# Chrissie-Law/Causal-Domain-Clustering-for-Multi-Domain-Recommendation

Measured on AMD Instinct MI355X. Metric: train samples/sec + AUC parity, PLE 3-domain batch 4096 at 1/2/4/8 MI355X, higher is better.
Workload: dtype bf16; 1 GPU; PLE 3-domain full training step (fwd + BCE + whole-table L2 + bwd + Adam), 26 fields x vocab 1000000, emb_dim=16, batch 4096/GPU; global_batch=4096, table_mode=lazy, hip_graph=True, row_sort_one_batch_ahead=True, id_dist=uniform, parallelism=dp1, attention_branch=False, full=False, steady_state=True, preroll_steps=1785, flush_every=64

## Files before the change

causal-domain-clustering-for-multi-domain-recommendation_amd/_lib.py:

```python
import ctypes as C
import os

from . import build as _build

MAX_GROUPS = 32
MAX_TENSORS = 48
MAX_GATES = 16
MAX_SEL = 16
MAX_BN_SEGS = 24
SORT_MAX_B = 16384
SORT_MAX_ROWS = 32768
BN_ROWS_PER_BLOCK = 64
ROWDOT_PARTS = 256
PREC_BF16 = 0
PREC_F32 = 1

c_f = C.c_float
c_i32 = C.c_int32
c_i64 = C.c_int64
c_p = C.c_void_p


class AdamHP(C.Structure):
    _fields_ = [("lerp_w", c_f), ("beta2", c_f), ("one_minus_beta2", c_f), ("eps", c_f),
# ... 317 lines not shown
    "cdc_embed_index": (c_i32, [c_p, c_p, c_p, c_p, c_i64, c_i32, c_i64, c_p]),
    "cdc_embed_sort_dedupe": (c_i32, [c_p, c_p, c_p, c_p, c_p, c_p, c_i64, c_i32, c_p]),
    "cdc_embed_sort_dedupe_ids": (c_i32, [c_p, c_p, c_i64, c_p, c_p, c_i32, c_p, c_p, c_p, c_p, c_p, c_p, c_i64, c_i32, c_p]),
    "cdc_embed_segment_sum": (c_i32, [c_p, c_p, c_p, c_p, c_p, c_p, c_i64, c_i32, c_i32, c_p]),
    "cdc_embed_segment_sum_direct": (c_i32, [c_p, c_p, c_p, c_p, c_p, c_p, c_i64, c_i32, c_i32, c_p]),
    "cdc_embed_segsum_lazy_update": (c_i32, [c_p, c_p, c_p, c_p, c_p, c_p, c_p, c_p, c_p, AdamHP, c_p, c_i64, c_i32, c_i32, c_i32, c_p]),
    "cdc_embed_grad_dense": (c_i32, [c_p, c_p, c_p, c_p, c_i64, c_i32, c_i32, c_i64, c_p]),
    "cdc_embed_adam_touched": (c_i32, [c_p, c_p, c_p, c_p, c_p, c_p, c_p, AdamHP, c_p, c_i64, c_i32, c_i32, c_p]),
    "cdc_embed_adam_dense_pass": (c_i32, [c_p, c_p, c_p, c_i64, AdamHP, c_p, c_p, c_p]),
    "cdc_embed_adam_patch": (c_i32, [c_p, c_p, c_p, c_p, c_p, c_p, c_i64, c_i32, c_i32, c_p]),
    "cdc_embed_lazy_catchup": (c_i32, [c_p, c_p, c_p, c_p, c_p, c_p, AdamHP, c_p, c_p, c_i32, c_i64, c_i32, c_i32, c_p]),
    "cdc_embed_lazy_catchup_gather": (c_i32, [c_p, c_p, c_p, c_p, c_p, c_p, c_p, c_p, AdamHP, c_p, c_p, c_p, c_i64, c_i64, c_i32, c_i32, c_p]),
    "cdc_embed_lazy_update": (c_i32, [c_p, c_p, c_p, c_p, c_p, c_p, c_p, AdamHP, c_p, c_p, c_i32, c_i64, c_i32, c_i32, c_p]),
    "cdc_embed_lazy_flush": (c_i32, [c_p, c_p, c_p, c_p, c_i64, c_i32, AdamHP, c_p, c_i32, c_i32, c_i32, c_i32, c_p]),
    "cdc_embed_lazy_flush_bg": (c_i32, [c_p, c_p, c_p, c_p, c_i64, c_i32, AdamHP, c_p, c_i32, c_i32, c_i32, c_i32, c_i32, c_p]),
    "cdc_embed_merge_dedupe": (c_i32, [c_p, c_p, c_p, c_p, c_p, c_p, c_i64, c_i32, c_i32, c_p]),
    "cdc_eval_workspace_bytes": (c_i64, [c_i64, c_i32]),
    "cdc_eval_metrics": (c_i32, [c_p, c_p, c_p, c_i64, c_i64, c_i32, c_p, c_p, c_p, c_p, c_i64, c_p]),
    "cdc_shard_bucket": (c_i32, [c_p, c_p, c_p, c_p, c_p, c_i64, c_i32, c_i32, c_i32, c_p]),
    "cdc_shard_expand": (c_i32, [c_p, c_p, c_p, c_p, c_p, c_p, c_p, c_i64, c_i32, c_i32, c_i32, c_i32, c_p]),
    "cdc_shard_pack": (c_i32, [c_p, c_p, c_p, c_p, c_p, c_i64, c_i32, c_i32, c_i32, c_i32, c_p]),
    "cdc_glinear_fwd": (c_i32, [C.POINTER(LinFwdArgs), c_i32, c_p]),
    "cdc_glinear_bwd_x": (c_i32, [C.POINTER(LinBwdxArgs), c_i32, c_p]),
    "cdc_transpose_multi": (c_i32, [C.POINTER(TransposeArgs), c_p]),
    "cdc_gemm_bf16_nt": (c_i32, [C.POINTER(G2Args), c_p]),
    "cdc_weight_shadows": (c_i32, [C.POINTER(WShadowArgs), c_p]),
    "cdc_shadow_bf16": (c_i32, [C.POINTER(ShadowArgs), c_p]),
    "cdc_glinear_bwd_w": (c_i32, [C.POINTER(LinBwdwArgs), c_i32, c_p]),
    "cdc_glinear_bwd_w_pair": (c_i32, [C.POINTER(LinBwdwArgs), C.POINTER(LinBwdwArgs), c_p, c_p]),
    "cdc_glinear_bwd_w_pair_reduce": (c_i32, [C.POINTER(LinBwdwArgs), C.POINTER(LinBwdwArgs), c_p, c_p]),
# ... 137 lines not shown
```

causal-domain-clustering-for-multi-domain-recommendation_amd/csrc/common.h:

```cpp
#pragma once
#include <hip/hip_runtime.h>
#include <stdint.h>
#include <stdio.h>
#include "cdcmdr.h"

#define CDC_WAVE 64

void cdc_set_error(const char* fmt, ...);

#define CDC_CHECK_ARG(cond, code, ...)            \
    do {                                          \
        if (!(cond)) {                            \
            cdc_set_error(__VA_ARGS__);           \
            return (code);                        \
        }                                         \
    } while (0)

#define CDC_LAUNCH_CHECK(name)                                                     \
    do {                                                                           \
        hipError_t e__ = hipGetLastError();                                        \
        if (e__ != hipSuccess) {                                                   \
            cdc_set_error("%s: launch failed: %s", name, hipGetErrorString(e__)); \
            return (int)e__;                                                       \
        }                                                                          \
// ... 111 lines not shown
        }
    }
}
__device__ __forceinline__ void adam_scaled_step_pk(cdc_f2& w, cdc_f2& M, cdc_f2& V, float beta1, float beta2, float C1, float C2) {
    M = __builtin_elementwise_fma((cdc_f2){beta1, beta1}, M, w);
    V = __builtin_elementwise_fma((cdc_f2){beta2, beta2}, V, w * w);
    cdc_f2 sq;
    sq.x = __builtin_amdgcn_sqrtf(V.x);
    sq.y = __builtin_amdgcn_sqrtf(V.y);
    const cdc_f2 d = __builtin_elementwise_fma(sq, (cdc_f2){C1, C1}, (cdc_f2){C2, C2});
    cdc_f2 r;
    r.x = __builtin_amdgcn_rcpf(d.x);
    r.y = __builtin_amdgcn_rcpf(d.y);
    w = __builtin_elementwise_fma(M, r, w);
}
template <int N>
__device__ __forceinline__ void adam_replay_wave_scaled(float (&w)[N], float (&m)[N], float (&v)[N], int from, int to, const cdc_adam_hp& hp) {
    static_assert(N % 2 == 0, "pairs of elements");
    const int last_i = hp.n_scalars - 1;
    const float A_conv = hp.replay_tab[2 * last_i], E_conv = hp.replay_tab[2 * last_i + 1];
    const float beta1 = 1.f - hp.lerp_w;
    int fmin = from < to ? from : to;
#pragma unroll
    for (int o = 32; o > 0; o >>= 1) {
        const int other = __shfl_xor(fmin, o, 64);
        fmin = other < fmin ? other : fmin;
    }
    fmin = __builtin_amdgcn_readfirstlane(fmin);
    if (fmin >= to) return;
    const float ik1 = hp.ik1, ik2 = hp.ik2;
    cdc_f2 W[N / 2], M[N / 2], V[N / 2];
#pragma unroll
    for (int k = 0; k < N / 2; ++k) {
        W[k] = (cdc_f2){w[2 * k], w[2 * k + 1]};
        M[k] = (cdc_f2){m[2 * k], m[2 * k + 1]} * ik1;
        V[k] = (cdc_f2){v[2 * k], v[2 * k + 1]} * ik2;
    }
    for (int s = fmin + 1; s <= to; ++s) {
        float A = A_conv, E = E_conv;
        if (s < last_i) { A = hp.replay_tab[2 * s]; E = hp.replay_tab[2 * s + 1]; }
        if (s > from) {
#pragma unroll
            for (int k = 0; k < N / 2; ++k) adam_scaled_step_pk(W[k], M[k], V[k], beta1, hp.beta2, A, E);
        }
    }
    if (from < to) {
#pragma unroll
        for (int k = 0; k < N / 2; ++k) {
            const cdc_f2 mo = __builtin_elementwise_fma(M[k], (cdc_f2){hp.k1, hp.k1}, M[k] * hp.k1_lo);
            const cdc_f2 vo = __builtin_elementwise_fma(V[k], (cdc_f2){hp.k2, hp.k2}, V[k] * hp.k2_lo);
            w[2 * k] = W[k].x; w[2 * k + 1] = W[k].y;
            m[2 * k] = mo.x; m[2 * k + 1] = mo.y;
            v[2 * k] = vo.x; v[2 * k + 1] = vo.y;
        }
    }
}

template <bool FAST, int N>
__device__ __forceinline__ void adam_replay_wave(float (&w)[N], float (&m)[N], float (&v)[N], int from, int to, const AdamConsts& c,
                                                 const cdc_adam_hp& hp) {
    if constexpr (FAST && N % 2 == 0) {
        if (hp.replay_tab && hp.k1 > 0.f && hp.k2 > 0.f) {
            adam_replay_wave_scaled<N>(w, m, v, from, to, hp);
            return;
        }
    }
    const int last_i = hp.n_scalars - 1;
    const float ss_conv = hp.step_scalars[2 * last_i];
    const float bc_conv = FAST ? hp.inv_bc2[last_i] : hp.step_scalars[2 * last_i + 1];
    int fmin = from < to ? from : to;
#pragma unroll
    for (int o = 32; o > 0; o >>= 1) {
        const int other = __shfl_xor(fmin, o, 64);
        fmin = other < fmin ? other : fmin;
    }
    fmin = __builtin_amdgcn_readfirstlane(fmin);
    for (int s = fmin + 1; s <= to; ++s) {
        float ss = ss_conv, bc = bc_conv;
        if (s < last_i) {
            ss = hp.step_scalars[2 * s];
            bc = FAST ? hp.inv_bc2[s] : hp.step_scalars[2 * s + 1];
        }
        if (s > from) {
            if constexpr (FAST && N % 2 == 0) {
#pragma unroll
                for (int k = 0; k < N; k += 2) {
                    cdc_f2 w2 = {w[k], w[k + 1]}, m2 = {m[k], m[k + 1]}, v2 = {v[k], v[k + 1]};
                    adam_elem_fast_pk(w2, m2, v2, c, ss, bc);
                    w[k] = w2.x; w[k + 1] = w2.y; m[k] = m2.x; m[k + 1] = m2.y; v[k] = v2.x; v[k + 1] = v2.y;
                }
            } else {
#pragma unroll
                for (int k = 0; k < N; ++k) {
                    if (FAST) adam_elem_fast(w[k], m[k], v[k], c, ss, bc);
                    else adam_elem(w[k], m[k], v[k], 0.f, c, ss, bc);
                }
            }
// ... 55 lines not shown
```

causal-domain-clustering-for-multi-domain-recommendation_amd/csrc/embedding.hip:

```cpp
#include "common.h"
#include "adam_dense.h"

template <int VEC>
__global__ void __launch_bounds__(256) k_gather_fwd(const int32_t* __restrict__ ids, const int32_t* __restrict__ offsets,
                                                    const float* __restrict__ table, float* __restrict__ out,
                                                    __bf16* __restrict__ out_h, int64_t ld_out_h,
                                                    int32_t* __restrict__ idx_out, int32_t* __restrict__ err_flag,
                                                    int64_t n_pos, int32_t F, int32_t D, int64_t R) {
    CDC_PRIO_MAIN();
    const int chunks = D / VEC;
    const int64_t total = n_pos * chunks;
    for (int64_t i = (int64_t)blockIdx.x * blockDim.x + threadIdx.x; i < total; i += (int64_t)gridDim.x * blockDim.x) {
        const int64_t pos = i / chunks;
        const int c = (int)(i - pos * chunks);
        const int f = (int)(pos % F);
        const int32_t row = (int32_t)((uint32_t)ids[pos] + (uint32_t)offsets[f]);
        const bool ok = row >= 0 && (int64_t)row < R;
        if (c == 0 && idx_out) idx_out[pos] = ok ? row : -1;
        if (!ok && c == 0 && err_flag) atomicMax(err_flag, (int32_t)(pos < 0x7ffffffe ? pos + 1 : 0x7fffffff));
        if (VEC == 4) {
            float4 val = make_float4(0.f, 0.f, 0.f, 0.f);
            if (ok) val = *reinterpret_cast<const float4*>(table + (int64_t)row * D + c * 4);
            *reinterpret_cast<float4*>(out + pos * D + c * 4) = val;
            if (out_h) {
// ... 1242 lines not shown
                  CDC_E_BADARG, "embed_lazy_update: null pointer");
    CDC_CHECK_ARG(B > 0 && F > 0 && D > 0, CDC_E_BADARG, "embed_lazy_update: bad sizes");
    const bool vec = (D % 4 == 0) && ((((uintptr_t)w | (uintptr_t)m | (uintptr_t)v | (uintptr_t)rowgrad) & 15) == 0);
    const int64_t total = (int64_t)F * B * (vec ? D / 4 : D);
    int blocks = (int)std::min<int64_t>(cdc_ceil_div(total, 256), 256 * 16);
    if (vec)
        hipLaunchKernelGGL(k_lazy_update<4>, dim3(blocks), dim3(256), 0, (hipStream_t)stream, rowgrad, uniq_row, uniq_cnt, w, m, v, last, hp,
                           step_dev, (int32_t)B, F, D);
    else
        hipLaunchKernelGGL(k_lazy_update<1>, dim3(blocks), dim3(256), 0, (hipStream_t)stream, rowgrad, uniq_row, uniq_cnt, w, m, v, last, hp,
                           step_dev, (int32_t)B, F, D);
    CDC_LAUNCH_CHECK("embed_lazy_update");
    return 0;
}

template <bool FAST, int VEC>
__global__ void __launch_bounds__(256) __attribute__((amdgpu_waves_per_eu(8, 8))) k_lazy_flush(float* __restrict__ w, float* __restrict__ m, float* __restrict__ v,
                                                    int32_t* __restrict__ last, int64_t R, int32_t D, cdc_adam_hp hp,
                                                    const int32_t* __restrict__ step_dev, int32_t step_bias, int32_t period,
                                                    int32_t own_mod, int32_t own_rem, int32_t mark, int64_t win_lo, int64_t win_n) {
    const int target = *step_dev + step_bias;
    int64_t row_lo = 0, row_hi = R;
    if (period > 1) {
        const int64_t rps = (R + period - 1) / period;
        row_lo = (int64_t)(((target % period) + period) % period) * rps;
        row_hi = row_lo + rps < R ? row_lo + rps : R;
        if (row_lo >= row_hi) return;
    }
    if (win_lo > row_lo) row_lo = win_lo;
    if (win_lo + win_n < row_hi) row_hi = win_lo + win_n;
    if (row_lo >= row_hi) return;
    const AdamConsts c = make_consts(hp);
    const int64_t stride = own_mod > 1 ? own_mod : 1;
    int64_t first = row_lo;
    if (stride > 1) first = row_lo + ((own_rem - row_lo % stride) + stride) % stride;
    if (first >= row_hi) return;
    const int64_t n_rows = (row_hi - first + stride - 1) / stride;
    const int chunks = D / VEC;
    const int64_t total = n_rows * chunks;
    typedef float f4v __attribute__((ext_vector_type(4)));
    const int32_t itotal = (int32_t)total;
    auto row_of = [&](int32_t i) -> int64_t { return first + (int64_t)(i / chunks) * stride; };
    auto fetch = [&](int32_t i, int& from, float (&wv)[VEC], float (&mv)[VEC], float (&vv)[VEC]) __attribute__((always_inline)) {
        const bool in = i < itotal;
        const int64_t row = in ? row_of(i) : first;
        from = in ? last[row] : target;
        const bool act = in && from < target;
        if (!act) from = target;
#pragma unroll
        for (int k = 0; k < VEC; ++k) { wv[k] = 0.f; mv[k] = 0.f; vv[k] = 1.f; }
        if (act) {
            const int64_t e0 = row * D + (i % chunks) * VEC;
            if (VEC == 4) {
                const f4v a4 = __builtin_nontemporal_load(reinterpret_cast<const f4v*>(w + e0)),
                          b4 = __builtin_nontemporal_load(reinterpret_cast<const f4v*>(m + e0)),
                          c4 = __builtin_nontemporal_load(reinterpret_cast<const f4v*>(v + e0));
#pragma unroll
                for (int k = 0; k < 4; ++k) { wv[k] = a4[k]; mv[k] = b4[k]; vv[k] = c4[k]; }
            } else {
                wv[0] = w[e0]; mv[0] = m[e0]; vv[0] = v[e0];
            }
        }
    };
    const int32_t gstride = (int32_t)(gridDim.x * blockDim.x);
    int cfrom, nfrom;
    float cw[VEC], cm[VEC], cv[VEC], nw[VEC], nm[VEC], nv[VEC];
    int32_t i = (int32_t)(blockIdx.x * blockDim.x + threadIdx.x);
    fetch(i, cfrom, cw, cm, cv);
    for (int32_t base = (int32_t)(blockIdx.x * blockDim.x); base < itotal; base += gstride, i += gstride) {
        fetch(base + gstride < itotal ? i + gstride : itotal, nfrom, nw, nm, nv);
        const bool act = cfrom < target;
        if (__any(act)) {
            adam_replay_wave<FAST, VEC>(cw, cm, cv, cfrom, target, c, hp);
            if (act) {
                const int64_t row = row_of(i);
                const int64_t e0 = row * D + (i % chunks) * VEC;
                if (VEC == 4) {
                    __builtin_nontemporal_store((f4v){cw[0], cw[1], cw[2], cw[3]}, reinterpret_cast<f4v*>(w + e0));
                    __builtin_nontemporal_store((f4v){cm[0], cm[1], cm[2], cm[3]}, reinterpret_cast<f4v*>(m + e0));
                    __builtin_nontemporal_store((f4v){cv[0], cv[1], cv[2], cv[3]}, reinterpret_cast<f4v*>(v + e0));
                } else {
                    w[e0] = cw[0]; m[e0] = cm[0]; v[e0] = cv[0];
                }
                if (mark && (i % chunks) == 0) last[row] = target;
            }
        }
        cfrom = nfrom;
#pragma unroll
        for (int k = 0; k < VEC; ++k) { cw[k] = nw[k]; cm[k] = nm[k]; cv[k] = nv[k]; }
    }
}
__global__ void __launch_bounds__(256) k_lazy_set_last(int32_t* __restrict__ last, int64_t R, const int32_t* __restrict__ step_dev,
                                                       int32_t step_bias, int32_t period, int32_t own_mod, int32_t own_rem) {
    const int target = *step_dev + step_bias;
    int64_t row_lo = 0, row_hi = R;
    if (period > 1) {
        const int64_t rps = (R + period - 1) / period;
        row_lo = (int64_t)(((target % period) + period) % period) * rps;
        row_hi = row_lo + rps < R ? row_lo + rps : R;
    }
    for (int64_t i = row_lo + (int64_t)blockIdx.x * blockDim.x + threadIdx.x; i < row_hi; i += (int64_t)gridDim.x * blockDim.x) {
        if (own_mod > 1 && (i % own_mod) != own_rem) continue;
        if (last[i] < target) last[i] = target;
    }
}

static int lazy_flush_launch(float* w, float* m, float* v, int32_t* last, int64_t R, int32_t D, cdc_adam_hp hp,
                             const int32_t* step_dev, int32_t step_bias, int32_t period, int32_t own_mod, int32_t own_rem,
                             int32_t waves_per_simd, void* stream) {
    CDC_CHECK_ARG(w && m && v && last && step_dev && hp.step_scalars && hp.n_scalars > 0, CDC_E_BADARG, "embed_lazy_flush: null pointer");
    CDC_CHECK_ARG(R > 0 && D > 0 && period >= 0 && own_mod >= 0 && (own_mod <= 1 || (own_rem >= 0 && own_rem < own_mod)), CDC_E_BADARG,
                  "embed_lazy_flush: bad sizes");
    CDC_CHECK_ARG(!hp.fast_replay || hp.inv_bc2, CDC_E_BADARG, "embed_lazy_flush: fast_replay needs the inv_bc2 table");
    const bool vec = (D % 4 == 0) && ((((uintptr_t)w | (uintptr_t)m | (uintptr_t)v) & 15) == 0);
    int64_t rows_call = period > 1 ? cdc_ceil_div(R, period) : R;
    if (own_mod > 1) rows_call = cdc_ceil_div(rows_call, own_mod) + 1;
    int blocks = (int)std::max<int64_t>(1, std::min<int64_t>(cdc_ceil_div(rows_call * D / (vec ? 4 : 1), 256), 256 * 16));
    if (waves_per_simd > 0) {
        static int n_cu = 0;
        if (n_cu == 0) {
            int dev = 0, v_ = 0;
            if (hipGetDevice(&dev) != hipSuccess || hipDeviceGetAttribute(&v_, hipDeviceAttributeMultiprocessorCount, dev) != hipSuccess || v_ <= 0) v_ = 256;
            n_cu = v_;
        }
        const int64_t cap = (int64_t)waves_per_simd * n_cu;
        if (blocks > cap) blocks = (int)cap;
    }
    hipStream_t st = (hipStream_t)stream;
    const int32_t chunks = vec ? D / 4 : D;
    const int32_t mark = (64 % chunks == 0) ? 1 : 0;
    const int64_t max_items = ((int64_t)1 << 31) - 1 - (int64_t)blocks * 256 - 256;
    const int64_t win_rows = std::max<int64_t>(1, max_items / chunks);
    CDC_CHECK_ARG(period <= 1 || rows_call <= win_rows, CDC_E_TOOBIG,
                  "embed_lazy_flush: a slice of %lld rows x %d chunks exceeds the 2^31 work items of one launch (raise flush_every)",
                  (long long)rows_call, (int)chunks);
    for (int64_t lo = 0; lo < R; lo += (period > 1 ? R : win_rows)) {
        const int64_t n = period > 1 ? R : std::min<int64_t>(win_rows, R - lo);
        if (hp.fast_replay) {
            if (vec) hipLaunchKernelGGL((k_lazy_flush<true, 4>), dim3(blocks), dim3(256), 0, st, w, m, v, last, R, D, hp, step_dev, step_bias, period, own_mod, own_rem, mark, lo, n);
            else     hipLaunchKernelGGL((k_lazy_flush<true, 1>), dim3(blocks), dim3(256), 0, st, w, m, v, last, R, D, hp, step_dev, step_bias, period, own_mod, own_rem, mark, lo, n);
        } else {
            if (vec) hipLaunchKernelGGL((k_lazy_flush<false, 4>), dim3(blocks), dim3(256), 0, st, w, m, v, last, R, D, hp, step_dev, step_bias, period, own_mod, own_rem, mark, lo, n);
            else     hipLaunchKernelGGL((k_lazy_flush<false, 1>), dim3(blocks), dim3(256), 0, st, w, m, v, last, R, D, hp, step_dev, step_bias, period, own_mod, own_rem, mark, lo, n);
        }
    }
    CDC_LAUNCH_CHECK("embed_lazy_flush");
    if (!mark) {
        int blocks2 = (int)std::max<int64_t>(1, std::min<int64_t>(cdc_ceil_div(period > 1 ? cdc_ceil_div(R, period) : R, 256), 256 * 16));
        hipLaunchKernelGGL(k_lazy_set_last, dim3(blocks2), dim3(256), 0, (hipStream_t)stream, last, R, step_dev, step_bias, period, own_mod, own_rem);
        CDC_LAUNCH_CHECK("embed_lazy_set_last");
    }
    return 0;
}
extern "C" int cdc_embed_lazy_flush(float* w, float* m, float* v, int32_t* last, int64_t R, int32_t D, cdc_adam_hp hp,
                                    const int32_t* step_dev, int32_t step_bias, int32_t period, int32_t own_mod, int32_t own_rem,
                                    void* stream) {
    return lazy_flush_launch(w, m, v, last, R, D, hp, step_dev, step_bias, period, own_mod, own_rem, 0, stream);
}
extern "C" int cdc_embed_lazy_flush_bg(float* w, float* m, float* v, int32_t* last, int64_t R, int32_t D, cdc_adam_hp hp,
                                       const int32_t* step_dev, int32_t step_bias, int32_t period, int32_t own_mod, int32_t own_rem,
                                       int32_t waves_per_simd, void* stream) {
    return lazy_flush_launch(w, m, v, last, R, D, hp, step_dev, step_bias, period, own_mod, own_rem, waves_per_simd, stream);
}


#define SHARD_MAX_RANKS 16
__global__ void __launch_bounds__(SORT_THREADS) k_shard_bucket(const int32_t* __restrict__ uniq_row, const int32_t* __restrict__ uniq_cnt,
                                                               int32_t* __restrict__ send_ids, int32_t* __restrict__ slot_of,
                                                               int32_t* __restrict__ overflow, int32_t B, int32_t F, int32_t n_rank,
                                                               int32_t cap) {
    __shared__ int32_t wave_tot[SORT_THREADS / 64];
    const int f = blockIdx.x, o = blockIdx.y, tid = threadIdx.x;
    const int n = uniq_cnt[f];
    const int per = (B + SORT_THREADS - 1) / SORT_THREADS;
    const int begin = tid * per;
    const int32_t* ur = uniq_row + (int64_t)f * B;
    int local = 0;
// ... 119 lines not shown
```

causal-domain-clustering-for-multi-domain-recommendation_amd/optim.py:

```python
import ctypes as C
import math

import os

import torch

from . import _lib as L


def step_scalar_table(lr, beta1, beta2, n=4096, truncate=False):
    rows = [(0.0, 1.0)]
    for t in range(1, n):
        rows.append((lr / (1.0 - beta1 ** t), math.sqrt(1.0 - beta2 ** t)))
    tab = torch.tensor(rows, dtype=torch.float64).to(torch.float32)
    if truncate:
        same = (tab == tab[-1]).all(dim=1)
        first = int(torch.nonzero(~same).max().item()) + 1 if bool((~same).any()) else 0
        tab = tab[:first + 1].contiguous()
    return tab


class FusedAdam:
    def __init__(self, model, lr=1e-3, betas=(0.9, 0.99), eps=1e-8, weight_decay=1e-8, table_mode="dense", frozen=(),
                 fast_replay=True, flush_every=64):
# ... 117 lines not shown
    def flush_slice(self, background_waves=0):
        if self.table_mode != "lazy" or self.flush_every <= 1:
            return
        nb = 24.0 * self.table.numel() / self.flush_every / max(self.own_mod, 1)
        if background_waves > 0:
            L.launch("cdc_embed_lazy_flush(slice)", self.lib.cdc_embed_lazy_flush_bg,
                     (self.table.data_ptr(), self.table_m.data_ptr(), self.table_v.data_ptr(), self.table_last.data_ptr(),
                      self.table.shape[0], self.table.shape[1], self._hp(), self.step_dev.data_ptr(), -1, self.flush_every,
                      self.own_mod, self.own_rem, int(background_waves)), self._stream(), nbytes=nb)
            return
        L.launch("cdc_embed_lazy_flush(slice)", self.lib.cdc_embed_lazy_flush,
                 (self.table.data_ptr(), self.table_m.data_ptr(), self.table_v.data_ptr(), self.table_last.data_ptr(),
                  self.table.shape[0], self.table.shape[1], self._hp(), self.step_dev.data_ptr(), -1, self.flush_every,
                  self.own_mod, self.own_rem), self._stream(), nbytes=nb)

    def catchup(self, B, F, D, tag=""):
        assert self.table_mode == "lazy"
        ws = self._workspace(B, F, D, tag)
        L.launch("cdc_embed_lazy_catchup", self.lib.cdc_embed_lazy_catchup,
                 (ws["uniq"].data_ptr(), ws["cnt"].data_ptr(), self.table.data_ptr(), self.table_m.data_ptr(),
                  self.table_v.data_ptr(), self.table_last.data_ptr(), self._hp(), self.step_dev.data_ptr(), None, 0, B, F, D), self._stream())

    def catchup_gather(self, B, F, D, tag, out_ptr, out_h, ld_out_h):
        assert self.table_mode == "lazy"
        ws = self._workspace(B, F, D, tag)
        L.launch("cdc_embed_lazy_catchup_gather", self.lib.cdc_embed_lazy_catchup_gather,
                 (ws["uniq"].data_ptr(), ws["cnt"].data_ptr(), ws["seg"].data_ptr(), ws["perm"].data_ptr(), self.table.data_ptr(),
                  self.table_m.data_ptr(), self.table_v.data_ptr(), self.table_last.data_ptr(), self._hp(), self.step_dev.data_ptr(),
                  out_ptr, out_h, ld_out_h, B, F, D), self._stream(), nbytes=float(B) * F * (D * 4 + 4 + D * 4))

# ... 191 lines not shown
```

causal-domain-clustering-for-multi-domain-recommendation_amd/trainer.py:

```python
import ctypes as C
import os

import torch

from . import _lib as L
from .optim import FusedAdam


def _run_steps(steps):
    def fn():
        st = C.c_void_p(torch.cuda.current_stream().cuda_stream)
        for s_ in steps:
            s_(st)
    return fn


def _merge_pieces(seq):
    merged = []
    for is_comm, fn in seq:
        if merged and not is_comm and not merged[-1][0]:
            merged[-1][1].append(fn)
        else:
            merged.append((is_comm, [fn]))
    return merged


class TrainStep:

    def __init__(self, model, optimizer: FusedAdam, batch_size, mode="multi", use_graph=False, dist=None, sync_bn=True,
                 table_dist=None, shard_slack=1.5, train_mode=True, overlap=True, overlap_waves=2, sort_ahead=True, fuse_gather=False,
                 defer_dw_reduce=None, global_rows=None, cap_rows=None, tower_one_launch=True, rows_dense_one_launch=True):
        self.model, self.opt, self.B, self.mode = model, optimizer, int(batch_size), mode
        self.lib = L.load()
        self.dist = dist
        self.sync_bn = bool(sync_bn)
        self.world = 1 if dist is None else dist.world_size
        self.dp_on = self.world > 1 or bool(getattr(dist, "force", False))
        self.global_B = self.B * self.world if global_rows is None else int(global_rows)
        self._shard_slack = float(shard_slack)
        dev = optimizer.device
        self.device = dev
        self.train_mode = bool(train_mode)
        self._overlap_ok, self._overlap_waves = bool(overlap), int(overlap_waves)
        self._rows_dense_one = bool(rows_dense_one_launch) and not self.dp_on
        self.tower_one_launch = bool(tower_one_launch)
        self._defer_dw = (not self.dp_on) if defer_dw_reduce is None else (bool(defer_dw_reduce) and not self.dp_on)
        assert mode in ("multi", "single", "mean", "star", "single_group")
        self.holder = self._build_plan()
        self.plan = self.holder.plan
        self.emb = self.holder.emb_op
        self.out = self.holder.outputs[0]
        self.y = torch.zeros(self.B, dtype=torch.int16, device=dev)
        self.group = torch.zeros(self.B, dtype=torch.int64, device=dev) if mode == "multi" else None
        if mode == "single_group":
            self.group_in = self.holder.inputs[1]
        if mode == "star":
            self.group = self.holder.inputs[1]
            self.order = self.holder.extra_outputs[0]
            self.y_perm = torch.zeros(self.B, dtype=torch.int16, device=dev)
# ... 175 lines not shown
            bg, fused = self._overlap_ok, self._fuse_gather_ok
            side = self._side_stream() if bg else main
            if bg:
                side.wait_stream(main)
            with torch.cuda.stream(side):
                if not have:
                    opt.begin_step_sort(emb.ids, emb.offsets, B, F, D, tag=cur, err=emb.err if fused else None, begin=False)
                if fused:
                    oh, ldh = plan.shadow_view(emb.out) if (plan.use_g2 and plan.has_shadow(emb.out)) else (None, 0)
                    opt.catchup_gather(B, F, D, cur, emb.out.ptr, oh, ldh)
                else:
                    opt.catchup(B, F, D, cur)
                if bg:
                    rows_ready = torch.cuda.Event()
                    rows_ready.record(side)
                opt.flush_slice(background_waves=self._overlap_waves if bg else 0)
                if prefetch:
                    opt.begin_step_sort(self.ids_next, emb.offsets, B, F, D, tag=nxt, begin=False)
            nws = plan.n_wshadow_steps
            for fn in plan.fwd_steps[:nws]:
                fn(st)
            if bg:
                main.wait_event(rows_ready)
            for fn in plan.fwd_steps[nws:]:
                if not (fused and fn is emb.fwd_step):
                    fn(st)
            self._bce()
            plan.backward()
            if self._rows_dense_one:
                if bg:
                    main.wait_stream(side)
                opt.rows_and_dense_step(emb.idx, emb.out.grad.root, B, F, D, plan.param_grads, plan._param_refs, plan.grad_slabs, tag=cur)
            else:
# ... 390 lines not shown
```

include/cdcmdr.h:

```cpp
#ifndef CDCMDR_H
#define CDCMDR_H

#include <stdint.h>

#ifdef __cplusplus
extern "C" {
#endif

#define CDC_ABI_VERSION 1

#define CDC_E_BADARG   (-1)
#define CDC_E_TOOBIG   (-2)
#define CDC_E_ALIGN    (-3)

#define CDC_PREC_BF16 0
#define CDC_PREC_F32  1

#define CDC_MAX_GROUPS 32
#define CDC_MAX_TENSORS 48

int cdc_abi_version(void);
const char* cdc_last_error(void);


// ... 52 lines not shown
                          float* w, float* m, float* v, int32_t* last,
                          cdc_adam_hp hp, const int32_t* step_dev, double* reg_ring, int32_t ring_len,
                          int64_t B, int32_t F, int32_t D, void* stream);
int cdc_embed_lazy_catchup_gather(const int32_t* uniq_row, const int32_t* uniq_cnt, const int32_t* seg_start, const int32_t* perm,
                                  float* w, float* m, float* v, int32_t* last, cdc_adam_hp hp, const int32_t* step_dev,
                                  float* out, void* out_h, int64_t ld_out_h, int64_t B, int32_t F, int32_t D, void* stream);
int cdc_embed_segsum_lazy_update(const float* d_out, const int32_t* seg_start, const int32_t* perm, const int32_t* uniq_cnt,
                                 const int32_t* uniq_row, float* w, float* m, float* v, int32_t* last, cdc_adam_hp hp,
                                 const int32_t* step_dev, int64_t B, int32_t F, int32_t D, int32_t short_only, void* stream);
int cdc_embed_lazy_flush(float* w, float* m, float* v, int32_t* last, int64_t R, int32_t D,
                         cdc_adam_hp hp, const int32_t* step_dev, int32_t step_bias, int32_t period,
                         int32_t own_mod, int32_t own_rem, void* stream);
int cdc_embed_lazy_flush_bg(float* w, float* m, float* v, int32_t* last, int64_t R, int32_t D,
                            cdc_adam_hp hp, const int32_t* step_dev, int32_t step_bias, int32_t period,
                            int32_t own_mod, int32_t own_rem, int32_t waves_per_simd, void* stream);

int cdc_embed_merge_dedupe(const int32_t* idx, int32_t* uniq_row, int32_t* seg_start, int32_t* perm, int32_t* uniq_cnt,
                           uint64_t* scratch, int64_t B, int32_t F, int32_t n_runs, void* stream);
int cdc_shard_bucket(const int32_t* uniq_row, const int32_t* uniq_cnt, int32_t* send_ids, int32_t* slot_of, int32_t* overflow,
                     int64_t B, int32_t F, int32_t n_rank, int32_t cap, void* stream);
int cdc_shard_expand(const float* rows_recv, const int32_t* uniq_row, const int32_t* uniq_cnt, const int32_t* seg_start,
                     const int32_t* perm, const int32_t* slot_of, float* out, int64_t B, int32_t F, int32_t D,
                     int32_t n_rank, int32_t cap, void* stream);
int cdc_shard_pack(const float* rowgrad, const int32_t* uniq_row, const int32_t* uniq_cnt, const int32_t* slot_of, float* send,
                   int64_t B, int32_t F, int32_t D, int32_t n_rank, int32_t cap, void* stream);

typedef struct {
    const float* x;  int64_t ldx;
    const float* w;  int64_t ldw;
    const float* bias;
// ... 652 lines not shown
```

Before: 13.10 million samples/s.

## Fuse next-batch sort/dedupe into the background lazy-flush kernel

Adds a combined kernel in which the first F blocks run a register/LDS bitonic sort-dedupe of the next batch's ids at raised priority, while the remaining blocks perform the background lazy Adam flush slice. The flush work is split proportionally between the sort blocks and the others. This replaces the separate flush and sort launches on the side stream. The intent is to save a launch and let the sort overlap the flush inside one grid. It also pins replay scalars to SGPRs and uses shift/mask indexing when chunks is a power of two. The cost is more code paths, a new bitonic sort implementation that must match the old one, and sort blocks that might unbalance the flush.

```diff
diff --git a/causal-domain-clustering-for-multi-domain-recommendation_amd/_lib.py b/causal-domain-clustering-for-multi-domain-recommendation_amd/_lib.py
--- a/causal-domain-clustering-for-multi-domain-recommendation_amd/_lib.py
+++ b/causal-domain-clustering-for-multi-domain-recommendation_amd/_lib.py
@@ -355,6 +355,8 @@
     "cdc_embed_lazy_update": (c_i32, [c_p, c_p, c_p, c_p, c_p, c_p, c_p, AdamHP, c_p, c_p, c_i32, c_i64, c_i32, c_i32, c_p]),
     "cdc_embed_lazy_flush": (c_i32, [c_p, c_p, c_p, c_p, c_i64, c_i32, AdamHP, c_p, c_i32, c_i32, c_i32, c_i32, c_p]),
     "cdc_embed_lazy_flush_bg": (c_i32, [c_p, c_p, c_p, c_p, c_i64, c_i32, AdamHP, c_p, c_i32, c_i32, c_i32, c_i32, c_i32, c_p]),
+    "cdc_embed_lazy_flush_bg_sort": (c_i32, [c_p, c_p, c_p, c_p, c_i64, c_i32, AdamHP, c_p, c_i32, c_i32, c_i32, c_i32, c_i32,
+                                             c_p, c_p, c_p, c_p, c_p, c_p, c_p, c_p, c_i64, c_i32, c_p]),
     "cdc_embed_merge_dedupe": (c_i32, [c_p, c_p, c_p, c_p, c_p, c_p, c_i64, c_i32, c_i32, c_p]),
     "cdc_eval_workspace_bytes": (c_i64, [c_i64, c_i32]),
     "cdc_eval_metrics": (c_i32, [c_p, c_p, c_p, c_i64, c_i64, c_i32, c_p, c_p, c_p, c_p, c_i64, c_p]),
diff --git a/causal-domain-clustering-for-multi-domain-recommendation_amd/csrc/common.h b/causal-domain-clustering-for-multi-domain-recommendation_amd/csrc/common.h
--- a/causal-domain-clustering-for-multi-domain-recommendation_amd/csrc/common.h
+++ b/causal-domain-clustering-for-multi-domain-recommendation_amd/csrc/common.h
@@ -149,7 +149,10 @@
     r.y = __builtin_amdgcn_rcpf(d.y);
     w = __builtin_elementwise_fma(M, r, w);
 }
-template <int N>
+__device__ __forceinline__ float uniform_sgpr(float x) {
+    return __builtin_bit_cast(float, __builtin_amdgcn_readfirstlane(__builtin_bit_cast(int, x)));
+}
+template <int N, bool PIN = false>
 __device__ __forceinline__ void adam_replay_wave_scaled(float (&w)[N], float (&m)[N], float (&v)[N], int from, int to, const cdc_adam_hp& hp) {
     static_assert(N % 2 == 0, "pairs of elements");
     const int last_i = hp.n_scalars - 1;
@@ -174,6 +177,7 @@
     for (int s = fmin + 1; s <= to; ++s) {
         float A = A_conv, E = E_conv;
         if (s < last_i) { A = hp.replay_tab[2 * s]; E = hp.replay_tab[2 * s + 1]; }
+        if constexpr (PIN) { A = uniform_sgpr(A); E = uniform_sgpr(E); }
         if (s > from) {
 #pragma unroll
             for (int k = 0; k < N / 2; ++k) adam_scaled_step_pk(W[k], M[k], V[k], beta1, hp.beta2, A, E);
@@ -191,12 +195,12 @@
     }
 }
 
-template <bool FAST, int N>
+template <bool FAST, int N, bool PIN = false>
 __device__ __forceinline__ void adam_replay_wave(float (&w)[N], float (&m)[N], float (&v)[N], int from, int to, const AdamConsts& c,
                                                  const cdc_adam_hp& hp) {
     if constexpr (FAST && N % 2 == 0) {
         if (hp.replay_tab && hp.k1 > 0.f && hp.k2 > 0.f) {
-            adam_replay_wave_scaled<N>(w, m, v, from, to, hp);
+            adam_replay_wave_scaled<N, PIN>(w, m, v, from, to, hp);
             return;
         }
     }
@@ -216,6 +220,7 @@
             ss = hp.step_scalars[2 * s];
             bc = FAST ? hp.inv_bc2[s] : hp.step_scalars[2 * s + 1];
         }
+        if constexpr (PIN) { ss = uniform_sgpr(ss); bc = uniform_sgpr(bc); }
         if (s > from) {
             if constexpr (FAST && N % 2 == 0) {
 #pragma unroll
diff --git a/causal-domain-clustering-for-multi-domain-recommendation_amd/csrc/embedding.hip b/causal-domain-clustering-for-multi-domain-recommendation_amd/csrc/embedding.hip
--- a/causal-domain-clustering-for-multi-domain-recommendation_amd/csrc/embedding.hip
+++ b/causal-domain-clustering-for-multi-domain-recommendation_amd/csrc/embedding.hip
@@ -1280,11 +1280,169 @@
     return 0;
 }
 
-template <bool FAST, int VEC>
+#ifndef RS_SHARE_NUM
+#define RS_SHARE_NUM 1
+#endif
+#define RS_SHARE_DEN 4
+#define RS_KPL 16
+#define RS_MAX_B (256 * RS_KPL)
+__device__ __forceinline__ bool rs_less(uint32_t ah, uint32_t al, uint32_t bh, uint32_t bl) {
+    return ah < bh || (ah == bh && al < bl);
+}
+__device__ __forceinline__ void rs_cmpex(uint32_t& ah, uint32_t& al, uint32_t& bh, uint32_t& bl, bool up) {
+    const bool sw = rs_less(bh, bl, ah, al) == up;
+    const uint32_t th = ah, tl = al;
+    ah = sw ? bh : ah; al = sw ? bl : al;
+    bh = sw ? th : bh; bl = sw ? tl : bl;
+}
+__device__ __forceinline__ void rs_keep(uint32_t& ah, uint32_t& al, uint32_t ph, uint32_t pl, bool keep_min) {
+    const bool take = rs_less(ph, pl, ah, al) == keep_min;
+    ah = take ? ph : ah; al = take ? pl : al;
+}
+template <int J, int K>
+__device__ __forceinline__ void rs_reg_stage(uint32_t (&kh)[RS_KPL], uint32_t (&kl)[RS_KPL], bool up) {
+#pragma unroll
+    for (int r = 0; r < RS_KPL; ++r)
+        if ((r & J) == 0) rs_cmpex(kh[r], kl[r], kh[r | J], kl[r | J], K > 0 ? ((r & K) == 0) == up : up);
+}
+__device__ __forceinline__ void rs_sort_dedupe(const SortSrc& src, int32_t* __restrict__ uniq_row, int32_t* __restrict__ seg_start,
+                                               int32_t* __restrict__ perm, int32_t* __restrict__ uniq_cnt, uint64_t* __restrict__ scratch,
+                                               int32_t B, int32_t F, int32_t n_sort, int32_t* s_row, int32_t* s_tot) {
+    const int f = blockIdx.x, tid = threadIdx.x, lane = tid & 63, wave = tid >> 6;
+    const int base = tid * RS_KPL;
+    uint32_t kh[RS_KPL], kl[RS_KPL];
+    const uint32_t off = (uint32_t)src.offsets[f];
+    int32_t bad = 0;
+#pragma unroll
+    for (int r = 0; r < RS_KPL; ++r) {
+        const int i = base + r;
+        const uint32_t pos = (uint32_t)(i < B ? i : 0) * (uint32_t)F + (uint32_t)f;
+        const int32_t row = (int32_t)((uint32_t)src.idx[pos] + off);
+        const bool ok = row >= 0 && (int64_t)row < src.R;
+        if (i < B && !ok) bad = (int32_t)pos + 1;
+        kh[r] = (i < B && ok) ? (uint32_t)row : 0xffffffffu;
+        kl[r] = i < B ? (uint32_t)i : 0xffffffffu;
+    }
+    if (bad && src.err_flag) atomicMax(src.err_flag, bad);
+    rs_reg_stage<1, 2>(kh, kl, true);
+    rs_reg_stage<2, 4>(kh, kl, true);
+    rs_reg_stage<1, 4>(kh, kl, true);
+    rs_reg_stage<4, 8>(kh, kl, true);
+    rs_reg_stage<2, 8>(kh, kl, true);
+    rs_reg_stage<1, 8>(kh, kl, true);
+    uint32_t* xh = reinterpret_cast<uint32_t*>(scratch + (int64_t)f * 2 * B);
+    uint32_t* xl = xh + n_sort;
+    for (int k = 16; k <= n_sort; k <<= 1) {
+        const bool up = (base & k) == 0;
+        for (int j = k >> 1; j >= 1024; j >>= 1) {
+            const int wm = j >> 10;
+            uint32_t me = tid;
+            asm volatile("" : "+v"(me));
+            const uint32_t nl = (uint32_t)n_sort >> 4;
+            if (me < nl) {
+#pragma unroll
+                for (int r = 0; r < RS_KPL; ++r) { xh[r * nl + me] = kh[r]; xl[r * nl + me] = kl[r]; }
+            }
+            __syncthreads();
+            if (me < nl) {
+                const bool keep_min = ((wave & wm) == 0) == up;
+                const uint32_t pt = me ^ (uint32_t)(wm << 6);
+#pragma unroll
+                for (int r = 0; r < RS_KPL; ++r) rs_keep(kh[r], kl[r], xh[r * nl + pt], xl[r * nl + pt], keep_min);
+            }
+            __syncthreads();
+        }
+        for (int j = (k >> 1) < 512 ? (k >> 1) : 512; j >= 16; j >>= 1) {
+            const int lm = j >> 4;
+            const bool keep_min = ((lane & lm) == 0) == up;
+            const int src_lane = (lane ^ lm) << 2;
+#pragma unroll
+            for (int g = 0; g < RS_KPL; g += 4) {
+                uint32_t ph[4], pl[4];
+#pragma unroll
+                for (int r = 0; r < 4; ++r) {
+                    ph[r] = (uint32_t)__builtin_amdgcn_ds_bpermute(src_lane, (int)kh[g + r]);
+                    pl[r] = (uint32_t)__builtin_amdgcn_ds_bpermute(src_lane, (int)kl[g + r]);
+                }
+                __builtin_amdgcn_sched_barrier(0);
+#pragma unroll
+                for (int r = 0; r < 4; ++r) rs_keep(kh[g + r], kl[g + r], ph[r], pl[r], keep_min);
+            }
+        }
+        rs_reg_stage<8, 0>(kh, kl, up);
+        rs_reg_stage<4, 0>(kh, kl, up);
+        rs_reg_stage<2, 0>(kh, kl, up);
+        rs_reg_stage<1, 0>(kh, kl, up);
+    }
+    int dbase = base;
+    asm volatile("" : "+v"(dbase));
+    uint32_t prev = (uint32_t)__shfl_up((int)kh[RS_KPL - 1], 1, 64);
+    if (lane == 63) s_row[wave] = (int32_t)kh[RS_KPL - 1];
+    uint32_t head_mask = 0;
+#pragma unroll
+    for (int r = 1; r < RS_KPL; ++r)
+        if (kh[r] != kh[r - 1] && dbase + r < B) head_mask |= 1u << r;
+    __syncthreads();
+    if (lane == 0 && wave > 0) prev = (uint32_t)s_row[wave - 1];
+    if (dbase < B && (dbase == 0 || kh[0] != prev)) head_mask |= 1u;
+    const int local = __popc(head_mask);
+    int inc = local;
+#pragma unroll
+    for (int o = 1; o < 64; o <<= 1) {
+        const int t = __shfl_up(inc, o, 64);
+        if (lane >= o) inc += t;
+    }
+    if (lane == 63) s_tot[wave] = inc;
+    __syncthreads();
+    int u = inc - local, total = 0;
+#pragma unroll
+    for (int wv = 0; wv < 4; ++wv) {
+        const int t = s_tot[wv];
+        u += wv < wave ? t : 0;
+        total += t;
+    }
+    int32_t* urow = uniq_row + (int64_t)f * B;
+    int32_t* sst = seg_start + (int64_t)f * (B + 1);
+    int32_t* prm = perm + (int64_t)f * B;
+#pragma unroll
+    for (int r = 0; r < RS_KPL; ++r) {
+        const int i = dbase + r;
+        if (i < B) {
+            if ((head_mask >> r) & 1u) {
+                urow[u] = (int32_t)kh[r];
+                sst[u] = i;
+                ++u;
+            }
+            prm[i] = (int32_t)kl[r];
+        }
+    }
+    if (tid == 0) {
+        sst[total] = B;
+        uniq_cnt[f] = total;
+    }
+}
+struct SliceSort {
+    SortSrc src;
+    int32_t *uniq_row, *seg_start, *perm, *uniq_cnt;
+    uint64_t* scratch;
+    int32_t B, F, n_sort;
+};
+template <bool FAST, int VEC, bool SORT>
 __global__ void __launch_bounds__(256) __attribute__((amdgpu_waves_per_eu(8, 8))) k_lazy_flush(float* __restrict__ w, float* __restrict__ m, float* __restrict__ v,
                                                     int32_t* __restrict__ last, int64_t R, int32_t D, cdc_adam_hp hp,
                                                     const int32_t* __restrict__ step_dev, int32_t step_bias, int32_t period,
-                                                    int32_t own_mod, int32_t own_rem, int32_t mark, int64_t win_lo, int64_t win_n) {
+                                                    int32_t own_mod, int32_t own_rem, int32_t mark, int64_t win_lo, int64_t win_n,
+                                                    const SliceSort ss) {
+    if constexpr (SORT) {
+        __shared__ int32_t s_x[8];
+        if ((int32_t)blockIdx.x < ss.F) {
+            __builtin_amdgcn_s_setprio(1);
+            rs_sort_dedupe(ss.src, ss.uniq_row, ss.seg_start, ss.perm, ss.uniq_cnt, ss.scratch, ss.B, ss.F, ss.n_sort, s_x, s_x + 4);
+            __builtin_amdgcn_s_setprio(0);
+        }
+        asm volatile("s_waitcnt vmcnt(0) lgkmcnt(0)" ::: "memory");
+        __builtin_amdgcn_sched_barrier(0);
+    }
     const int target = *step_dev + step_bias;
     int64_t row_lo = 0, row_hi = R;
     if (period > 1) {
@@ -1305,8 +1463,21 @@
     const int chunks = D / VEC;
     const int64_t total = n_rows * chunks;
     typedef float f4v __attribute__((ext_vector_type(4)));
-    const int32_t itotal = (int32_t)total;
-    auto row_of = [&](int32_t i) -> int64_t { return first + (int64_t)(i / chunks) * stride; };
+    uint32_t blk = blockIdx.x, nblk = gridDim.x;
+    int32_t ilo = 0, iend = (int32_t)total;
+    if constexpr (SORT) {
+        const uint32_t tiles = ((uint32_t)iend + 255u) >> 8;
+        const uint32_t w_sort = (uint32_t)ss.F * RS_SHARE_NUM, w_all = w_sort + (nblk - (uint32_t)ss.F) * RS_SHARE_DEN;
+        const uint32_t split_t = tiles - tiles * w_sort / w_all;
+        const int32_t split = split_t < tiles ? (int32_t)(split_t << 8) : iend;
+        if (blk < (uint32_t)ss.F) { ilo = split; nblk = ss.F; }
+        else                      { iend = split; blk -= ss.F; nblk -= ss.F; }
+    }
+    const int32_t itotal = iend;
+    const int csh = SORT ? 31 - __builtin_clz((unsigned)chunks) : 0;
+    auto cdiv = [&](int32_t i) -> int32_t { if constexpr (SORT) return i >> csh; else return i / chunks; };
+    auto cmod = [&](int32_t i) -> int32_t { if constexpr (SORT) return i & (chunks - 1); else return i % chunks; };
+    auto row_of = [&](int32_t i) -> int64_t { return first + (int64_t)cdiv(i) * stride; };
     auto fetch = [&](int32_t i, int& from, float (&wv)[VEC], float (&mv)[VEC], float (&vv)[VEC]) __attribute__((always_inline)) {
         const bool in = i < itotal;
         const int64_t row = in ? row_of(i) : first;
@@ -1316,7 +1487,7 @@
 #pragma unroll
         for (int k = 0; k < VEC; ++k) { wv[k] = 0.f; mv[k] = 0.f; vv[k] = 1.f; }
         if (act) {
-            const int64_t e0 = row * D + (i % chunks) * VEC;
+            const int64_t e0 = row * D + cmod(i) * VEC;
             if (VEC == 4) {
                 const f4v a4 = __builtin_nontemporal_load(reinterpret_cast<const f4v*>(w + e0)),
                           b4 = __builtin_nontemporal_load(reinterpret_cast<const f4v*>(m + e0)),
@@ -1328,19 +1499,19 @@
             }
         }
     };
-    const int32_t gstride = (int32_t)(gridDim.x * blockDim.x);
+    const int32_t gstride = (int32_t)(nblk * blockDim.x);
     int cfrom, nfrom;
     float cw[VEC], cm[VEC], cv[VEC], nw[VEC], nm[VEC], nv[VEC];
-    int32_t i = (int32_t)(blockIdx.x * blockDim.x + threadIdx.x);
+    int32_t i = ilo + (int32_t)(blk * blockDim.x + threadIdx.x);
     fetch(i, cfrom, cw, cm, cv);
-    for (int32_t base = (int32_t)(blockIdx.x * blockDim.x); base < itotal; base += gstride, i += gstride) {
+    for (int32_t base = ilo + (int32_t)(blk * blockDim.x); base < itotal; base += gstride, i += gstride) {
         fetch(base + gstride < itotal ? i + gstride : itotal, nfrom, nw, nm, nv);
         const bool act = cfrom < target;
         if (__any(act)) {
-            adam_replay_wave<FAST, VEC>(cw, cm, cv, cfrom, target, c, hp);
+            adam_replay_wave<FAST, VEC, SORT>(cw, cm, cv, cfrom, target, c, hp);
             if (act) {
                 const int64_t row = row_of(i);
-                const int64_t e0 = row * D + (i % chunks) * VEC;
+                const int64_t e0 = row * D + cmod(i) * VEC;
                 if (VEC == 4) {
                     __builtin_nontemporal_store((f4v){cw[0], cw[1], cw[2], cw[3]}, reinterpret_cast<f4v*>(w + e0));
                     __builtin_nontemporal_store((f4v){cm[0], cm[1], cm[2], cm[3]}, reinterpret_cast<f4v*>(m + e0));
@@ -1348,7 +1519,9 @@
                 } else {
                     w[e0] = cw[0]; m[e0] = cm[0]; v[e0] = cv[0];
                 }
-                if (mark && (i % chunks) == 0) last[row] = target;
+                int tmark = target;
+                if constexpr (SORT) asm volatile("" : "+s"(tmark));
+                if (mark && cmod(i) == 0) last[row] = tmark;
             }
         }
         cfrom = nfrom;
@@ -1371,14 +1544,7 @@
     }
 }
 
-static int lazy_flush_launch(float* w, float* m, float* v, int32_t* last, int64_t R, int32_t D, cdc_adam_hp hp,
-                             const int32_t* step_dev, int32_t step_bias, int32_t period, int32_t own_mod, int32_t own_rem,
-                             int32_t waves_per_simd, void* stream) {
-    CDC_CHECK_ARG(w && m && v && last && step_dev && hp.step_scalars && hp.n_scalars > 0, CDC_E_BADARG, "embed_lazy_flush: null pointer");
-    CDC_CHECK_ARG(R > 0 && D > 0 && period >= 0 && own_mod >= 0 && (own_mod <= 1 || (own_rem >= 0 && own_rem < own_mod)), CDC_E_BADARG,
-                  "embed_lazy_flush: bad sizes");
-    CDC_CHECK_ARG(!hp.fast_replay || hp.inv_bc2, CDC_E_BADARG, "embed_lazy_flush: fast_replay needs the inv_bc2 table");
-    const bool vec = (D % 4 == 0) && ((((uintptr_t)w | (uintptr_t)m | (uintptr_t)v) & 15) == 0);
+static int lazy_flush_blocks(int64_t R, int32_t D, bool vec, int32_t period, int32_t own_mod, int32_t waves_per_simd, int64_t* rows_call_out) {
     int64_t rows_call = period > 1 ? cdc_ceil_div(R, period) : R;
     if (own_mod > 1) rows_call = cdc_ceil_div(rows_call, own_mod) + 1;
     int blocks = (int)std::max<int64_t>(1, std::min<int64_t>(cdc_ceil_div(rows_call * D / (vec ? 4 : 1), 256), 256 * 16));
@@ -1392,6 +1558,19 @@
         const int64_t cap = (int64_t)waves_per_simd * n_cu;
         if (blocks > cap) blocks = (int)cap;
     }
+    *rows_call_out = rows_call;
+    return blocks;
+}
+static int lazy_flush_launch(float* w, float* m, float* v, int32_t* last, int64_t R, int32_t D, cdc_adam_hp hp,
+                             const int32_t* step_dev, int32_t step_bias, int32_t period, int32_t own_mod, int32_t own_rem,
+                             int32_t waves_per_simd, void* stream) {
+    CDC_CHECK_ARG(w && m && v && last && step_dev && hp.step_scalars && hp.n_scalars > 0, CDC_E_BADARG, "embed_lazy_flush: null pointer");
+    CDC_CHECK_ARG(R > 0 && D > 0 && period >= 0 && own_mod >= 0 && (own_mod <= 1 || (own_rem >= 0 && own_rem < own_mod)), CDC_E_BADARG,
+                  "embed_lazy_flush: bad sizes");
+    CDC_CHECK_ARG(!hp.fast_replay || hp.inv_bc2, CDC_E_BADARG, "embed_lazy_flush: fast_replay needs the inv_bc2 table");
+    const bool vec = (D % 4 == 0) && ((((uintptr_t)w | (uintptr_t)m | (uintptr_t)v) & 15) == 0);
+    int64_t rows_call;
+    const int blocks = lazy_flush_blocks(R, D, vec, period, own_mod, waves_per_simd, &rows_call);
     hipStream_t st = (hipStream_t)stream;
     const int32_t chunks = vec ? D / 4 : D;
     const int32_t mark = (64 % chunks == 0) ? 1 : 0;
@@ -1403,11 +1582,11 @@
     for (int64_t lo = 0; lo < R; lo += (period > 1 ? R : win_rows)) {
         const int64_t n = period > 1 ? R : std::min<int64_t>(win_rows, R - lo);
         if (hp.fast_replay) {
-            if (vec) hipLaunchKernelGGL((k_lazy_flush<true, 4>), dim3(blocks), dim3(256), 0, st, w, m, v, last, R, D, hp, step_dev, step_bias, period, own_mod, own_rem, mark, lo, n);
-            else     hipLaunchKernelGGL((k_lazy_flush<true, 1>), dim3(blocks), dim3(256), 0, st, w, m, v, last, R, D, hp, step_dev, step_bias, period, own_mod, own_rem, mark, lo, n);
+            if (vec) hipLaunchKernelGGL((k_lazy_flush<true, 4, false>), dim3(blocks), dim3(256), 0, st, w, m, v, last, R, D, hp, step_dev, step_bias, period, own_mod, own_rem, mark, lo, n, SliceSort{});
+            else     hipLaunchKernelGGL((k_lazy_flush<true, 1, false>), dim3(blocks), dim3(256), 0, st, w, m, v, last, R, D, hp, step_dev, step_bias, period, own_mod, own_rem, mark, lo, n, SliceSort{});
         } else {
-            if (vec) hipLaunchKernelGGL((k_lazy_flush<false, 4>), dim3(blocks), dim3(256), 0, st, w, m, v, last, R, D, hp, step_dev, step_bias, period, own_mod, own_rem, mark, lo, n);
-            else     hipLaunchKernelGGL((k_lazy_flush<false, 1>), dim3(blocks), dim3(256), 0, st, w, m, v, last, R, D, hp, step_dev, step_bias, period, own_mod, own_rem, mark, lo, n);
+            if (vec) hipLaunchKernelGGL((k_lazy_flush<false, 4, false>), dim3(blocks), dim3(256), 0, st, w, m, v, last, R, D, hp, step_dev, step_bias, period, own_mod, own_rem, mark, lo, n, SliceSort{});
+            else     hipLaunchKernelGGL((k_lazy_flush<false, 1, false>), dim3(blocks), dim3(256), 0, st, w, m, v, last, R, D, hp, step_dev, step_bias, period, own_mod, own_rem, mark, lo, n, SliceSort{});
         }
     }
     CDC_LAUNCH_CHECK("embed_lazy_flush");
@@ -1427,6 +1606,46 @@
                                        const int32_t* step_dev, int32_t step_bias, int32_t period, int32_t own_mod, int32_t own_rem,
                                        int32_t waves_per_simd, void* stream) {
     return lazy_flush_launch(w, m, v, last, R, D, hp, step_dev, step_bias, period, own_mod, own_rem, waves_per_simd, stream);
+}
+extern "C" int cdc_embed_lazy_flush_bg_sort(float* w, float* m, float* v, int32_t* last, int64_t R, int32_t D, cdc_adam_hp hp,
+                                            const int32_t* step_dev, int32_t step_bias, int32_t period, int32_t own_mod, int32_t own_rem,
+                                            int32_t waves_per_simd, const int32_t* ids, const int32_t* offsets, int32_t* err_flag,
+                                            int32_t* uniq_row, int32_t* seg_start, int32_t* perm, int32_t* uniq_cnt, uint64_t* scratch,
+                                            int64_t B, int32_t F, void* stream) {
+    CDC_CHECK_ARG(w && m && v && last && step_dev && hp.step_scalars && hp.n_scalars > 0, CDC_E_BADARG, "embed_lazy_flush_bg_sort: null pointer");
+    CDC_CHECK_ARG(R > 0 && D > 0 && period >= 0 && own_mod >= 0 && (own_mod <= 1 || (own_rem >= 0 && own_rem < own_mod)), CDC_E_BADARG,
+                  "embed_lazy_flush_bg_sort: bad sizes");
+    CDC_CHECK_ARG(!hp.fast_replay || hp.inv_bc2, CDC_E_BADARG, "embed_lazy_flush_bg_sort: fast_replay needs the inv_bc2 table");
+    CDC_CHECK_ARG(ids && offsets && uniq_row && seg_start && perm && uniq_cnt, CDC_E_BADARG, "embed_lazy_flush_bg_sort: null pointer");
+    CDC_CHECK_ARG(B > 0 && F > 0, CDC_E_BADARG, "embed_lazy_flush_bg_sort: bad sizes");
+    CDC_CHECK_ARG(B <= CDC_SORT_MAX_ROWS, CDC_E_TOOBIG, "embed_lazy_flush_bg_sort: B=%ld exceeds %d", (long)B, CDC_SORT_MAX_ROWS);
+    CDC_CHECK_ARG(scratch || B <= SORT_CHUNK, CDC_E_BADARG, "embed_lazy_flush_bg_sort: B > %d needs a scratch buffer of 2*F*B uint64", SORT_CHUNK);
+    const bool vec = (D % 4 == 0) && ((((uintptr_t)w | (uintptr_t)m | (uintptr_t)v) & 15) == 0);
+    int64_t rows_call;
+    const int blocks = lazy_flush_blocks(R, D, vec, period, own_mod, waves_per_simd, &rows_call);
+    const int32_t chunks = vec ? D / 4 : D;
+    const bool one = vec && (64 % chunks == 0) && period > 1 &&
+                     rows_call * chunks <= ((int64_t)1 << 31) - 1 - (int64_t)blocks * 256 - 256 &&
+                     B <= RS_MAX_B && (B <= 1024 || scratch) && F < blocks && (int64_t)B * F < 0x7ffffffe &&
+                     (cdc_ceil_div(rows_call * chunks, 256) + 1) * F * RS_SHARE_NUM < ((int64_t)1 << 32);
+    if (!one) {
+        const int rc = lazy_flush_launch(w, m, v, last, R, D, hp, step_dev, step_bias, period, own_mod, own_rem, waves_per_simd, stream);
+        if (rc != 0) return rc;
+        const SortSrc src = {ids, offsets, R, nullptr, nullptr, 0, err_flag};
+        return sort_dedupe_launch(src, uniq_row, seg_start, perm, uniq_cnt, scratch, B, F, stream);
+    }
+    const SortSrc src = {ids, offsets, R, nullptr, nullptr, 0, err_flag};
+    const int32_t n_sort = B <= 1024 ? 1024 : (B <= 2048 ? 2048 : RS_MAX_B);
+    const SliceSort ss = {src, uniq_row, seg_start, perm, uniq_cnt, scratch, (int32_t)B, F, n_sort};
+    hipStream_t st = (hipStream_t)stream;
+    if (hp.fast_replay)
+        hipLaunchKernelGGL((k_lazy_flush<true, 4, true>), dim3(blocks), dim3(256), 0, st, w, m, v, last, R, D, hp, step_dev, step_bias, period, own_mod,
+                           own_rem, 1, (int64_t)0, R, ss);
+    else
+        hipLaunchKernelGGL((k_lazy_flush<false, 4, true>), dim3(blocks), dim3(256), 0, st, w, m, v, last, R, D, hp, step_dev, step_bias, period, own_mod,
+                           own_rem, 1, (int64_t)0, R, ss);
+    CDC_LAUNCH_CHECK("embed_lazy_flush_bg_sort");
+    return 0;
 }
 
 
diff --git a/causal-domain-clustering-for-multi-domain-recommendation_amd/optim.py b/causal-domain-clustering-for-multi-domain-recommendation_amd/optim.py
--- a/causal-domain-clustering-for-multi-domain-recommendation_amd/optim.py
+++ b/causal-domain-clustering-for-multi-domain-recommendation_amd/optim.py
@@ -155,6 +155,21 @@
                   self.table.shape[0], self.table.shape[1], self._hp(), self.step_dev.data_ptr(), -1, self.flush_every,
                   self.own_mod, self.own_rem), self._stream(), nbytes=nb)
 
+    def flush_slice_sort(self, background_waves, ids, offsets, B, F, D, tag="", err=None):
+        if self.table_mode != "lazy" or self.flush_every <= 1 or background_waves <= 0:
+            self.flush_slice(background_waves)
+            return self.begin_step_sort(ids, offsets, B, F, D, tag=tag, err=err, begin=False)
+        ws = self._workspace(B, F, D, tag)
+        nb = 24.0 * self.table.numel() / self.flush_every / max(self.own_mod, 1)
+        L.launch("cdc_embed_lazy_flush(slice)", self.lib.cdc_embed_lazy_flush_bg_sort,
+                 (self.table.data_ptr(), self.table_m.data_ptr(), self.table_v.data_ptr(), self.table_last.data_ptr(),
+                  self.table.shape[0], self.table.shape[1], self._hp(), self.step_dev.data_ptr(), -1, self.flush_every,
+                  self.own_mod, self.own_rem, int(background_waves),
+                  ids.data_ptr(), offsets.data_ptr(), None if err is None else err.data_ptr(),
+                  ws["uniq"].data_ptr(), ws["seg"].data_ptr(), ws["perm"].data_ptr(), ws["cnt"].data_ptr(),
+                  None if ws["scratch"] is None else ws["scratch"].data_ptr(), B, F), self._stream(), nbytes=nb)
+        return ws
+
     def catchup(self, B, F, D, tag=""):
         assert self.table_mode == "lazy"
         ws = self._workspace(B, F, D, tag)
diff --git a/causal-domain-clustering-for-multi-domain-recommendation_amd/trainer.py b/causal-domain-clustering-for-multi-domain-recommendation_amd/trainer.py
--- a/causal-domain-clustering-for-multi-domain-recommendation_amd/trainer.py
+++ b/causal-domain-clustering-for-multi-domain-recommendation_amd/trainer.py
@@ -29,7 +29,8 @@
 
     def __init__(self, model, optimizer: FusedAdam, batch_size, mode="multi", use_graph=False, dist=None, sync_bn=True,
                  table_dist=None, shard_slack=1.5, train_mode=True, overlap=True, overlap_waves=2, sort_ahead=True, fuse_gather=False,
-                 defer_dw_reduce=None, global_rows=None, cap_rows=None, tower_one_launch=True, rows_dense_one_launch=True):
+                 defer_dw_reduce=None, global_rows=None, cap_rows=None, tower_one_launch=True, rows_dense_one_launch=True,
+                 sort_in_slice=True):
         self.model, self.opt, self.B, self.mode = model, optimizer, int(batch_size), mode
         self.lib = L.load()
         self.dist = dist
@@ -43,6 +44,7 @@
         self.train_mode = bool(train_mode)
         self._overlap_ok, self._overlap_waves = bool(overlap), int(overlap_waves)
         self._rows_dense_one = bool(rows_dense_one_launch) and not self.dp_on
+        self._sort_in_slice = bool(sort_in_slice)
         self.tower_one_launch = bool(tower_one_launch)
         self._defer_dw = (not self.dp_on) if defer_dw_reduce is None else (bool(defer_dw_reduce) and not self.dp_on)
         assert mode in ("multi", "single", "mean", "star", "single_group")
@@ -248,9 +250,12 @@
                 if bg:
                     rows_ready = torch.cuda.Event()
                     rows_ready.record(side)
-                opt.flush_slice(background_waves=self._overlap_waves if bg else 0)
-                if prefetch:
-                    opt.begin_step_sort(self.ids_next, emb.offsets, B, F, D, tag=nxt, begin=False)
+                if bg and prefetch and not fused and self._sort_in_slice:
+                    opt.flush_slice_sort(self._overlap_waves, self.ids_next, emb.offsets, B, F, D, tag=nxt)
+                else:
+                    opt.flush_slice(background_waves=self._overlap_waves if bg else 0)
+                    if prefetch:
+                        opt.begin_step_sort(self.ids_next, emb.offsets, B, F, D, tag=nxt, begin=False)
             nws = plan.n_wshadow_steps
             for fn in plan.fwd_steps[:nws]:
                 fn(st)
diff --git a/include/cdcmdr.h b/include/cdcmdr.h
--- a/include/cdcmdr.h
+++ b/include/cdcmdr.h
@@ -90,6 +90,12 @@
 int cdc_embed_lazy_flush_bg(float* w, float* m, float* v, int32_t* last, int64_t R, int32_t D,
                             cdc_adam_hp hp, const int32_t* step_dev, int32_t step_bias, int32_t period,
                             int32_t own_mod, int32_t own_rem, int32_t waves_per_simd, void* stream);
+int cdc_embed_lazy_flush_bg_sort(float* w, float* m, float* v, int32_t* last, int64_t R, int32_t D,
+                                 cdc_adam_hp hp, const int32_t* step_dev, int32_t step_bias, int32_t period,
+                                 int32_t own_mod, int32_t own_rem, int32_t waves_per_simd,
+                                 const int32_t* ids, const int32_t* offsets, int32_t* err_flag, int32_t* uniq_row,
+                                 int32_t* seg_start, int32_t* perm, int32_t* uniq_cnt, uint64_t* scratch, int64_t B, int32_t F,
+                                 void* stream);
 
 int cdc_embed_merge_dedupe(const int32_t* idx, int32_t* uniq_row, int32_t* seg_start, int32_t* perm, int32_t* uniq_cnt,
                            uint64_t* scratch, int64_t B, int32_t F, int32_t n_runs, void* stream);
```

After: 13.35 million samples/s (median of 6 runs). 1.9% higher.
